# ecmwf-ifs/ecwam

Measured on AMD Instinct MI355X. Metric: grid-point spectral steps/sec (whole node) at O320, 36dir x 36freq, higher is better.
Workload: dtype f32; 1 GPU; O320 all-ocean octahedral grid, 421080 sea points, 36 dir x 36 freq (NFRE_RED=36), full WAMINTGR step = PROPAGS2 advection + NEWWIND + IMPLSCH as one kernel (PROPAGS2 inside IMPLSCH's tile load), IDELT=IDELPRO=450 s, flag set A (IPHYS=1, ISNONLIN=0, LLGCBZ0=F, LLNORMAGAM=F); points_per_gpu=421080, halo_points=0, parallelism=sea-point block x1, ranks=1

## Files before the change

__graft_entry__.py:

```python
from __future__ import annotations

import os
import sys

ROOT = os.path.dirname(os.path.abspath(__file__))
if ROOT not in sys.path:
    sys.path.insert(0, ROOT)


def build() -> None:
    from ecwam_amd import build as b

    lib = b.build()
    assert os.path.exists(lib)
    assert os.path.exists(b.build(variant="ctustrict"))
    assert os.path.exists(b.build(variant="nolead"))
    assert os.path.exists(b.build(variant="notrim"))
    for exe in b.build_fortran():
        assert os.path.exists(exe)
    from oracle import oracle

    oracle.build()
    from oracle import ref_build

    ref_build.build()
    sys.path.insert(0, os.path.join(ROOT, "tests"))
    try:
        import v2lib

        v2lib.build()
    except Exception as e:
        print(f"[build] tests/csrc second implementation not built: {e}", file=sys.stderr)
    import ecwam_amd
    from ecwam_amd import lib as L

    h = L.load()
    for name in L.EXPORTS + L.EXPORTS_START + L.EXPORTS_FORCING + L.EXPORTS_GRIBOUT + L.EXPORTS_GRIBIN:
        getattr(h, name)


def smoke() -> None:
    import numpy as np
    import torch

    sys.path.insert(0, os.path.join(ROOT, "tests"))
    from ecwam_amd import grid as G
    from ecwam_amd.tables import Config
    from ecwam_amd.wamintgr import Wamintgr
    from oracle.oracle import Oracle

    assert torch.cuda.is_available(), "smoke() needs a GPU"
    prec = "sp"
    cfg = Config(nang=36, nfre=36, nfre_red=36, idelt=450, idelpro=450)
    g = G.build_grid(12, mask="continents")
    m = Wamintgr(cfg, g, prec, device=0)
    m.init_synthetic(seed=4)
    assert m.build_weights() == 0 and m.fused_available()
    n = g.nsea
    fl = m.fl1.cpu().numpy().copy()
    wv = m.wvprpt.cpu().numpy()
    ff = m.ff.cpu().numpy()[:, :14].copy()
    env = m.ff.cpu().numpy()[:, 14:16].copy()
    o = Oracle(cfg, prec)
    m.step(fused=True)
    torch.cuda.synchronize()
    f3 = o.propags2(g, fl, o.ctu_weights(g, m.cgroup_ext.cpu().numpy(), float(cfg.idelpro)))
    f3[:, :, cfg.nfre_red:] = fl[:, :, cfg.nfre_red:]
    r = o.implsch(f3[:n], wv[:, 0], wv[:, 1], wv[:, 2], wv[:, 3], wv[:, 4], env, ff, np.zeros((n, 15), np.float32))
    got = m.fl1.cpu().numpy()[:n].astype(np.float64)
    want = r["FL1"].astype(np.float64)
    assert np.isfinite(got).all()
    same = m.mij.cpu().numpy() == r["MIJ"]
    assert same.mean() > 0.99
    peak = np.abs(want).max(axis=(1, 2), keepdims=True)
    err = (np.abs(got - want) / peak)[same].max()
    dfim = np.asarray(m.t.DFIM, dtype=np.float64)
    hs_g, hs_w = (4 * np.sqrt((x.sum(1) * dfim).sum(1)) for x in (got, want))
    e_hs = np.max(np.abs(hs_g - hs_w) / np.maximum(hs_w, 1e-12))
    assert err < 3e-5 and e_hs < 2e-6, (err, e_hs)
    print(f"smoke ok: {n} sea points, one WAMINTGR step as one kernel, max bin error {err:.2e} of the spectral peak, swh {e_hs:.2e}")
    m.ctx.close()


if __name__ == "__main__":
    build()
    if "--smoke" in sys.argv:
        smoke()
```

ecwam_amd/build.py:

```python
from __future__ import annotations

import hashlib
import os
import re
import shutil
import subprocess
import sys

HERE = os.path.dirname(os.path.abspath(__file__))
CSRC = os.path.join(HERE, "csrc")
LIBDIR = os.path.join(HERE, "lib")
LIB = os.path.join(LIBDIR, "libecwam_hip.so")
SOURCES = ["capi.hip", "propag.hip", "implsch4.hip", "implsch4a.hip", "implsch4x.hip", "implsch4r.hip", "implsch4rd.hip", "implsch4w.hip", "outbs.hip", "outbs_sep.hip", "outbs_ext.hip", "outbs_fl2nd.hip", "outbs_2nd.hip", "outbs_int.hip", "outblock.hip", "nest.hip", "start.hip", "forcing.hip", "gribout.hip", "gribin.hip"]
DERIVED = {"implsch4r.hip": ("implsch4r.hip", ["-DV4R_PREC=1"]), "implsch4rd.hip": ("implsch4r.hip", ["-DV4R_PREC=2"])}
HIPCC = shutil.which("hipcc") or "/opt/rocm/bin/hipcc"
FAST_DIV = ["-fno-hip-fp32-correctly-rounded-divide-sqrt"]
FLAGS = ["--offload-arch=gfx950", "-O3", "-fPIC", "-std=c++17", "-Wall", "-Wno-unused-variable", "-Wno-unused-but-set-variable"]
IMPLSCH_SOURCES = ("implsch4.hip", "implsch4a.hip", "implsch4x.hip", "implsch4r.hip", "implsch4rd.hip", "implsch4w.hip")
VARIANTS = {"": FAST_DIV, "exactdiv": ["-DECWAM_HIP_STRICT=0"], "strict1": ["-DECWAM_HIP_STRICT=1"], "strict2": FAST_DIV + ["-DECWAM_HIP_STRICT=2"],
            "site4": ["-DECWAM_HIP_STRICT=4"], "site8": ["-DECWAM_HIP_STRICT=8"], "site32": ["-DECWAM_HIP_STRICT=32"],
            "strict3": ["-DECWAM_HIP_STRICT=3"], "strict7": ["-DECWAM_HIP_STRICT=3", "-ffp-contract=off"],
            "noieee": FAST_DIV + ["-mno-amdgpu-ieee", "-fno-honor-nans"],
            "ctustrict": FAST_DIV,
            "nolead": FAST_DIV + ["-DV4_SINPUT_LEAD=0"],
            "notrim": FAST_DIV + ["-DV4_ONCE_TRIM=0"],
            "advO1": FAST_DIV + ["-O1"]}
VARIANT_ANY = {"ctustrict": ["-DECWAM_HIP_CTU_STRICT=1"]}
VARIANT_SOURCES = {"ctustrict": ("propag.hip", "implsch4a.hip"), "advO1": ("implsch4a.hip",)}

INCLUDE = os.path.join(HERE, "..", "include", "ecwam_hip.h")


def lib_path(variant: str = "") -> str:
    return LIB if not variant else os.path.join(LIBDIR, f"libecwam_hip_{variant}.so")


def _closure(path: str, seen: dict) -> None:
    path = os.path.normpath(path)
    if path in seen or not os.path.exists(path):
        return
    with open(path, "rb") as fh:
        data = fh.read()
    seen[path] = data
    for m in re.finditer(rb'^[ \t]*#[ \t]*include[ \t]*"([^"]+)"', data, re.M):
        _closure(os.path.join(os.path.dirname(path), m.group(1).decode()), seen)


def _stamp(src: str, flags: list) -> str:
    seen: dict = {}
    _closure(os.path.join(CSRC, src), seen)
    h = hashlib.sha256(" ".join([HIPCC, *flags]).encode())
    for k in sorted(seen):
        h.update(os.path.relpath(k, HERE).encode())
        h.update(seen[k])
    return h.hexdigest()


def build(force: bool = False, verbose: bool = False, variant: str = "") -> str:
    if variant not in VARIANTS:
        raise ValueError(f"unknown build variant {variant!r}: {sorted(VARIANTS)}")
    os.makedirs(LIBDIR, exist_ok=True)
    lib = lib_path(variant)
    objs, procs, stamps = [], [], {}
    for src in SOURCES:
        special = bool(variant) and src in VARIANT_SOURCES.get(variant, IMPLSCH_SOURCES)
        obj = os.path.join(LIBDIR, src.replace(".hip", f".{variant}.o" if special else ".o"))
        real_src, extra = DERIVED.get(src, (src, []))
        flags = FLAGS + extra + ((VARIANTS[variant] if special else FAST_DIV) if src in IMPLSCH_SOURCES else []) + (VARIANT_ANY.get(variant, []) if special else [])
        objs.append(obj)
        st = _stamp(real_src, flags)
        old = ""
        if os.path.exists(obj) and os.path.exists(obj + ".stamp"):
            with open(obj + ".stamp") as fh:
                old = fh.read().strip()
        if not force and old == st:
            continue
        stamps[obj] = st
        cmd = [HIPCC, *flags, f"-cuid=ecwam_{os.path.basename(obj).replace('.', '_')}", "-c", os.path.join(CSRC, real_src), "-o", obj]
        if verbose:
            print(" ".join(cmd), flush=True)
        procs.append((src, obj, subprocess.Popen(cmd, stdout=subprocess.PIPE, stderr=subprocess.STDOUT, text=True)))
    for src, obj, p in procs:
        out, _ = p.communicate()
        if p.returncode != 0:
            raise RuntimeError(f"hipcc failed for {src}:\n{out}")
        with open(obj + ".stamp", "w") as fh:
            fh.write(stamps[obj])
        if verbose and out.strip():
            print(out)
    link_stamp = hashlib.sha256("".join(open(o + ".stamp").read() for o in objs).encode()).hexdigest()
    if not procs and os.path.exists(lib) and os.path.exists(lib + ".stamp") and open(lib + ".stamp").read().strip() == link_stamp:
        return lib
    cmd = [HIPCC, "--offload-arch=gfx950", "-shared", "-fPIC", "-Wl,--no-undefined", "-o", lib, *objs]
    r = subprocess.run(cmd, stdout=subprocess.PIPE, stderr=subprocess.STDOUT, text=True)
    if r.returncode != 0:
        raise RuntimeError(f"link failed:\n{r.stdout}")
    with open(lib + ".stamp", "w") as fh:
        fh.write(link_stamp)
    return lib


FLANG = shutil.which("amdflang") or "/opt/rocm/lib/llvm/bin/flang"
FSRC = os.path.join(HERE, "fortran")
FFILES = ["ecwam_hip_capi.F90", "yowdrvtype_hip.F90", "ecwam_hip_mod.F90", "ecwam_hip_restart.F90", "wamintgr_hip.F90", "harness_case.F90"]
FPROGS = {"smoke_wamintgr_hip": "smoke_wamintgr_hip.F90", "seam_sequence": "seam_sequence.F90"}


def fortran_exe(prec: str, prog: str = "smoke_wamintgr_hip") -> str:
    return os.path.join(LIBDIR, f"{prog}_{prec}")


def build_fortran(force: bool = False) -> list:
    build(force=False)
    out = []
    for prec in ("sp", "dp"):
        exes = [fortran_exe(prec, p) for p in FPROGS]
        out += exes
        srcs = [os.path.join(FSRC, f) for f in FFILES + list(FPROGS.values())]
        if not force and all(os.path.exists(e) and all(os.path.getmtime(s) < os.path.getmtime(e) for s in srcs + [LIB]) for e in exes):
            continue
        moddir = os.path.join(LIBDIR, f"fmod_{prec}")
        os.makedirs(moddir, exist_ok=True)
        defs = ["-DECWAM_HIP_SINGLE"] if prec == "sp" else []

        def compile_(s):
            o = os.path.join(moddir, os.path.basename(s).replace(".F90", ".o"))
            r = subprocess.run([FLANG, "-cpp", "-O2", "-fPIC", *defs, "-module-dir", moddir, "-I", moddir, "-c", s, "-o", o],
                               stdout=subprocess.PIPE, stderr=subprocess.STDOUT, text=True)
            if r.returncode != 0:
                raise RuntimeError(f"flang failed for {s}:\n{r.stdout}")
            return o

        objs = [compile_(os.path.join(FSRC, f)) for f in FFILES]
        for prog, f in FPROGS.items():
            po = compile_(os.path.join(FSRC, f))
            r = subprocess.run([FLANG, "-o", fortran_exe(prec, prog), po, *objs, "-L", LIBDIR, "-lecwam_hip", f"-Wl,-rpath,{LIBDIR}", "-Wl,-rpath,$ORIGIN"],
                               stdout=subprocess.PIPE, stderr=subprocess.STDOUT, text=True)
            if r.returncode != 0:
                raise RuntimeError(f"fortran link failed ({prog}):\n{r.stdout}")
    return out


if __name__ == "__main__":
    vs = [a.split("=", 1)[1] for a in sys.argv[1:] if a.startswith("--variant=")]
    for v in vs or [""]:
        print(build(force="--force" in sys.argv, verbose=True, variant=v))
    if not vs:
        print(build_fortran(force="--force" in sys.argv))
```

ecwam_amd/csrc/implsch_v4.h:

```cpp
#pragma once
#include "ctu.h"

#define V4_NFRE 36
#ifdef ECWAM_HIP_DIAGNOSTICS
#define V4_PHASE_EXIT(k) do { if (tb.DBG_SKIP == (k)) return; } while (0)
#else
#define V4_PHASE_EXIT(k) do { } while (0)
#endif
#if defined(V4_CHECK) && V4_CHECK
#include <cassert>
#define V4_CHK(c) assert(c)
#else
#define V4_CHK(c) do { } while (0)
#endif
#ifndef V4_SINPUT_LEAD
#define V4_SINPUT_LEAD 1
#endif
#ifndef V4_ONCE_TRIM
#define V4_ONCE_TRIM 1
#endif
#define V4_NSTG 4
#define V4_NS(nang) ((V4_NFRE + (nang) / 2 - 1) / ((nang) / 2))
#define V4_PLN(pp, nang) ((pp) * ((nang) > V4_NFRE ? (nang) : V4_NFRE))
#define V4_NFAC 6

#define V4SYNC() WSYNC()
#define V4_WPE_MIN(T) (sizeof(T) == 4 ? 2 : 1)

template <typename T>
using V2 = T __attribute__((ext_vector_type(2)));

enum { FIN_AIRD = 0, FIN_UFRIC, FIN_Z0M, FIN_MIJ, FIN_XS, FIN_YS, FIN_F1DCOS3, FIN_F1DCOS2, FIN_F1DSIN2, FIN_F1D, FIN_RNFAC, FIN_PHIWA,
       FIN_SINWD, FIN_COSWD, FIN_WSWAVE, FIN_CICOVER, FIN_PHILF, FIN_XSTRESS, FIN_YSTRESS, FIN_Z0B, FIN_CHRNCK, FIN_COSDIFF, FIN_EMEAN, FIN_F1MEAN,
       FIN_TAUICX, FIN_TAUICY, FIN_STRNMS,
       FIN_W3RT,
       FIN_FMEAN, FIN_FMEANWS, FIN_AKMEAN, FIN_XKMEAN, FIN_SDS, FIN_SC, V4_NFIN = 36 };

__device__ __forceinline__ float v4_bp(int addr, float v) { return __int_as_float(__builtin_amdgcn_ds_bpermute(addr, __float_as_int(v))); }
__device__ __forceinline__ double v4_bp(int addr, double v) {
  const int lo = __builtin_amdgcn_ds_bpermute(addr, __double2loint(v));
  const int hi = __builtin_amdgcn_ds_bpermute(addr, __double2hiint(v));
  return __hiloint2double(hi, lo);
}
template <typename T>
__device__ __forceinline__ V2<T> v4_same(V2<T> v, int addr) {
  V2<T> r;
  r.x = v4_bp(addr, v.x);
  r.y = v4_bp(addr, v.y);
  return r;
}
template <typename T>
struct V4Rot { int a0, a1, a2, a3, a4; T fold; };
template <int CTRL>
__device__ __forceinline__ float v4_dpp(float v) {
  return __int_as_float(__builtin_amdgcn_update_dpp(0, __float_as_int(v), CTRL, 0xf, 0xf, true));
}
template <int CTRL>
__device__ __forceinline__ double v4_dpp(double v) {
  const int lo = __builtin_amdgcn_update_dpp(0, __double2loint(v), CTRL, 0xf, 0xf, true);
  const int hi = __builtin_amdgcn_update_dpp(0, __double2hiint(v), CTRL, 0xf, 0xf, true);
  return __hiloint2double(hi, lo);
}
#define V4_ROW_ROR(n) (0x120 + (n))
template <typename T>
__device__ __forceinline__ V2<T> v4_rowsum(V2<T> v) {
  T x = v.x, y = v.y;
  x += v4_dpp<V4_ROW_ROR(8)>(x); y += v4_dpp<V4_ROW_ROR(8)>(y);
  x += v4_dpp<V4_ROW_ROR(4)>(x); y += v4_dpp<V4_ROW_ROR(4)>(y);
  x += v4_dpp<V4_ROW_ROR(2)>(x); y += v4_dpp<V4_ROW_ROR(2)>(y);
  x += v4_dpp<V4_ROW_ROR(1)>(x); y += v4_dpp<V4_ROW_ROR(1)>(y);
  return V2<T>{x, y};
}
template <typename T>
__device__ __forceinline__ T v4_rowmax(T v) {
  v = m_max(v, v4_dpp<V4_ROW_ROR(8)>(v));
  v = m_max(v, v4_dpp<V4_ROW_ROR(4)>(v));
  v = m_max(v, v4_dpp<V4_ROW_ROR(2)>(v));
  v = m_max(v, v4_dpp<V4_ROW_ROR(1)>(v));
  return v;
}
template <>
__device__ __forceinline__ float v4_rowmax<float>(float v) {
  asm volatile("s_nop 1\n\tv_max_f32_dpp %0, %0, %0 row_ror:8 row_mask:0xf bank_mask:0xf bound_ctrl:1\n\t"
               "s_nop 1\n\tv_max_f32_dpp %0, %0, %0 row_ror:4 row_mask:0xf bank_mask:0xf bound_ctrl:1\n\t"
               "s_nop 1\n\tv_max_f32_dpp %0, %0, %0 row_ror:2 row_mask:0xf bank_mask:0xf bound_ctrl:1\n\t"
               "s_nop 1\n\tv_max_f32_dpp %0, %0, %0 row_ror:1 row_mask:0xf bank_mask:0xf bound_ctrl:1"
               : "+v"(v));
  return v;
}
template <int G, typename T>
__device__ __forceinline__ V2<T> v4_allsum(V2<T> v, const V4Rot<T>& r) {
  if constexpr (G == 18) {
    v = v + r.fold * v4_same<T>(v, r.a0);
    v = v4_rowsum<T>(v);
    return v4_same<T>(v, r.a1);
  } else {
    v = v + v4_same<T>(v, r.a0);
    if (G >= 12) v = v + v4_same<T>(v, r.a1);
    if (G == 24) v = v + v4_same<T>(v, r.a2);
    v = v + (v4_same<T>(v, r.a3) + v4_same<T>(v, r.a4));
    return v;
  }
}
template <int G, typename T>
__device__ __forceinline__ T v4_allsum1(T v, const V4Rot<T>& r) {
  if constexpr (G == 18) {
    v = v + r.fold * v4_bp(r.a0, v);
    v = v + v4_dpp<V4_ROW_ROR(8)>(v);
    v = v + v4_dpp<V4_ROW_ROR(4)>(v);
    v = v + v4_dpp<V4_ROW_ROR(2)>(v);
    v = v + v4_dpp<V4_ROW_ROR(1)>(v);
    return v4_bp(r.a1, v);
  } else {
    v = v + v4_bp(r.a0, v);
    if (G >= 12) v = v + v4_bp(r.a1, v);
    if (G == 24) v = v + v4_bp(r.a2, v);
    v = v + (v4_bp(r.a3, v) + v4_bp(r.a4, v));
    return v;
  }
}

template <int G, int N, int NB, typename T>
__device__ __forceinline__ void v4_allsum_n(T (&v)[N], const V4Rot<T>& r) {
  T e[N];
  if constexpr (G == 18) {
#pragma unroll
    for (int i = 0; i < N; i++) e[i] = v4_bp(r.a0, v[i]);
#pragma unroll
    for (int i = 0; i < N; i++) v[i] = v[i] + r.fold * e[i];
#pragma unroll
    for (int i = 0; i < N; i++) v[i] = v[i] + v4_dpp<V4_ROW_ROR(8)>(v[i]);
#pragma unroll
    for (int i = 0; i < N; i++) v[i] = v[i] + v4_dpp<V4_ROW_ROR(4)>(v[i]);
#pragma unroll
    for (int i = 0; i < N; i++) v[i] = v[i] + v4_dpp<V4_ROW_ROR(2)>(v[i]);
#pragma unroll
    for (int i = 0; i < N; i++) v[i] = v[i] + v4_dpp<V4_ROW_ROR(1)>(v[i]);
#pragma unroll
    for (int i = 0; i < NB; i++) e[i] = v4_bp(r.a1, v[i]);
#pragma unroll
    for (int i = 0; i < NB; i++) v[i] = e[i];
  } else {
#pragma unroll
    for (int i = 0; i < N; i++) e[i] = v4_bp(r.a0, v[i]);
#pragma unroll
    for (int i = 0; i < N; i++) v[i] = v[i] + e[i];
    if constexpr (G >= 12) {
#pragma unroll
      for (int i = 0; i < N; i++) e[i] = v4_bp(r.a1, v[i]);
#pragma unroll
      for (int i = 0; i < N; i++) v[i] = v[i] + e[i];
    }
    if constexpr (G == 24) {
#pragma unroll
      for (int i = 0; i < N; i++) e[i] = v4_bp(r.a2, v[i]);
#pragma unroll
      for (int i = 0; i < N; i++) v[i] = v[i] + e[i];
    }
    T f[N];
#pragma unroll
    for (int i = 0; i < N; i++) { e[i] = v4_bp(r.a3, v[i]); f[i] = v4_bp(r.a4, v[i]); }
#pragma unroll
    for (int i = 0; i < N; i++) v[i] = v[i] + (e[i] + f[i]);
  }
}

template <int G, typename T>
__device__ __forceinline__ T v4_allmax1(T v, const V4Rot<T>& r) {
  if constexpr (G == 18) {
    v = m_max(v, v4_bp(r.a0, v));
    v = v4_rowmax<T>(v);
    return v4_bp(r.a1, v);
  } else {
    v = m_max(v, v4_bp(r.a0, v));
    if (G >= 12) v = m_max(v, v4_bp(r.a1, v));
    if (G == 24) v = m_max(v, v4_bp(r.a2, v));
    return m_max(v, m_max(v4_bp(r.a3, v), v4_bp(r.a4, v)));
  }
}

template <int G, bool UNI, typename T>
__device__ __forceinline__ T v4_uni(T v, int p) {
  if constexpr (UNI && G != 18) return v4_bp(4 * (p * G), v);
  else return v;
}

template <int G, typename T, bool UNI = false>
__device__ __forceinline__ void v4_row_total_to_lds(T v, const V4Rot<T>& r, T* spw, int m, int p = 0) {
  if constexpr (G == 18) {
    v = v + r.fold * v4_bp(r.a0, v);
    v = v + v4_dpp<V4_ROW_ROR(8)>(v);
    v = v + v4_dpp<V4_ROW_ROR(4)>(v);
    v = v + v4_dpp<V4_ROW_ROR(2)>(v);
    v = v + v4_dpp<V4_ROW_ROR(1)>(v);
  } else {
    v = v4_allsum1<G, T>(v, r);
  }
  spw[m] = v4_uni<G, UNI>(v, p);
}

template <typename T, int NSH, int r>
__device__ __forceinline__ V2<T> v4_at(const T* row, const int (&sh)[2 * NSH + 1]) {
  if constexpr ((r & 1) == 0) {
    return *reinterpret_cast<const V2<T>*>(row + sh[r / 2 + NSH]);
  } else {
    return V2<T>{row[sh[(r - 1) / 2 + NSH] + 1], row[sh[(r + 1) / 2 + NSH]]};
  }
}

template <bool ON, typename T>
__device__ __forceinline__ T v4_vreg(T x) {
  if constexpr (ON && sizeof(T) == 4) {
    T r;
    asm("v_mov_b32 %0, %1" : "=v"(r) : "s"(x));
    return r;
  } else return x;
}
template <typename T>
__device__ __forceinline__ void v4_pin6(const T (&r)[6]) { asm volatile("" :: "s"(r[0]), "s"(r[1]), "s"(r[2]), "s"(r[3]), "s"(r[4]), "s"(r[5])); }
template <typename T>
__device__ __forceinline__ void v4_pin10(T (&r)[20], int o) {
  asm volatile("" :: "s"(r[o]), "s"(r[o + 1]), "s"(r[o + 2]), "s"(r[o + 3]), "s"(r[o + 4]), "s"(r[o + 5]), "s"(r[o + 6]), "s"(r[o + 7]), "s"(r[o + 8]), "s"(r[o + 9]));
}
template <typename T, int NSH, int ra, int rb>
__device__ __forceinline__ V2<T> v4_win(const T* row, const int (&sh)[2 * NSH + 1], V2<T> own, T ca, T cb) {
  static_assert(ra - rb == 1 || rb - ra == 1, "adjacent rotations");
  constexpr int lo = ra < rb ? ra : rb;
  constexpr int e = (lo >= 0) ? (lo / 2) * 2 : -(((-lo) + 1) / 2) * 2;
  static_assert(e / 2 + NSH >= 0 && e / 2 + 1 + NSH <= 2 * NSH, "shift table");
  const V2<T> a = (e == 0) ? own : *reinterpret_cast<const V2<T>*>(row + sh[e / 2 + NSH]);
  const V2<T> b = (e + 2 == 0) ? own : *reinterpret_cast<const V2<T>*>(row + sh[e / 2 + 1 + NSH]);
  const T el[4] = {a.x, a.y, b.x, b.y};
  return V2<T>{ca * el[ra - e] + cb * el[rb - e], ca * el[ra - e + 1] + cb * el[rb - e + 1]};
}

template <typename T, int NSH, int r>
__device__ __forceinline__ V2<T> v4_pair(const V2<T> (&A)[2 * NSH + 1]) {
  static_assert(r >= -2 * NSH && r <= 2 * NSH, "window");
  if constexpr ((r & 1) == 0) return A[NSH + r / 2];
  else return __builtin_shufflevector(A[NSH + (r - 1) / 2], A[NSH + (r + 1) / 2], 1, 2);
}
template <typename T, int NSH, int NH, int d>
__device__ __forceinline__ void v4_sat_taps(const V2<T> (&A)[2 * NSH + 1], const T (&wt)[NH + 1], V2<T>& acc) {
  if constexpr (d <= NH) {
    acc += wt[NH - d] * (v4_pair<T, NSH, -d>(A) + v4_pair<T, NSH, d>(A));
    v4_sat_taps<T, NSH, NH, d + 1>(A, wt, acc);
  }
}

template <typename T, int PP, bool RARE>
__device__ __forceinline__ void v4_stresso(const DevTab<T>& tb, T* sSC, int lane, bool LLPHIWA) {
  if constexpr (PP <= 3) {
    stresso_stage<T, PP, RARE>(tb, sSC, lane, LLPHIWA);
  } else {
    stresso_stage<T, 3, RARE>(tb, sSC, lane, LLPHIWA);
    WSYNC();
    v4_stresso<T, PP - 3, RARE>(tb, sSC + 3 * NSC, lane, LLPHIWA);
  }
}

template <typename T, int NANG_, int PP_>
struct V4Ctx {
  int lane, p, j;
  T* tile;
  int own;
  T* fac4;
  T* sq;
  T* zcn;
  T* c;
  V4Rot<T> rot;
  V2<T> sinth, costh;
  T rDFIM, rDFIMOFR, rDFIMFR, rZPIFR, rRHOWG, rCOFRM4, rFLMAX;
};
enum { Q4_BSC = 0, Q4_SBO, Q4_CINV, Q4_WAVNUM };

template <typename T>
struct V4Adv {
  const T* f_in;
  const int* klon;
  const int* klat;
  const int* kcor;
  const T* cg;
  const T* pt;
  const T* dirT;
  const int* dirI;
  T xdella, delpro;
  const T* gin;
  T delpro_lf;
  int gin_k, mlf;
  const T* obs;
  int m0, m1;
};
template <typename T, int NANG, int PP, int MODE, int NSCR>
__device__ __forceinline__ void v4_advect_tile(const V4Adv<T>& A, int ij0, int n, int lane, T* __restrict__ sT, T* __restrict__ sScr) {
  constexpr int NFRE = V4_NFRE, N = NANG * NFRE, RS = PP * NANG, VEC = 16 / (int)sizeof(T), NC = NFRE / VEC, NVL = N / VEC;
  constexpr int NFULL = NVL / 64, NREM = NVL - 64 * NFULL, NTS = (PP * NREM + 63) / 64, NCH = NFULL * PP + NTS, NRND = NFULL + NTS, D = 3;
  constexpr int PTW = 20;
  typedef T VT __attribute__((ext_vector_type(VEC)));
  typedef int I4 __attribute__((ext_vector_type(4)));
  T* sB = sScr;
  T* sPt = sB + PP * 5 * NFRE;
  T* sK = sPt + PP * PTW;
  constexpr bool LF = (MODE & 3) == 3;
  constexpr bool OBS = (MODE & 4) != 0;
  constexpr int NB = OBS ? 11 : 8;
  static_assert(MODE & 1, "modes: 1 plain, 3 fast waves, + 4 obstructions");
  constexpr int NKW = NANG * 4 + 4 + (LF ? NANG * 2 : 0);
  int* sI = reinterpret_cast<int*>(sK + NKW);
  int* sD = sI + PP * 16;
  static_assert((PP * 5 * NFRE + PP * PTW + NKW) * sizeof(T) + (PP * 16 + NANG * 4) * sizeof(int) <= NSCR * sizeof(T), "LDS scratch of the advecting load");
  for (int i = lane; i < PP * PTW; i += 64) {
    const int q = i / PTW, e = i - q * PTW;
    const T* g = A.pt + (size_t)(ij0 + (q < n ? q : n - 1)) * 12;
    T v = T(0);
    if (e < 12) v = g[e];
    else if (e < 18) v = T(1) - g[e - 6];
    else if (e == 18) v = g[0] * g[2];
    else v = A.xdella * g[2];
    if (e == 1) v = m_abs(v);
    sPt[i] = v;
  }
  for (int i = lane; i < PP * 16; i += 64) {
    const int q = i >> 4, e = i & 15;
    const int ijq = ij0 + (q < n ? q : n - 1);
    int v = ijq;
    if (e >= 1 && e <= 2) v = A.klon[(size_t)ijq * 2 + (e - 1)];
    if (e >= 3 && e <= 6) v = A.klat[(size_t)ijq * 4 + (e - 3)];
    if (e >= 7 && e <= 14) v = A.kcor[(size_t)ijq * 8 + (e - 7)];
    sI[i] = v;
  }
  for (int i = lane; i < NKW; i += 64) {
// ... 187 lines not shown
      const T ZLOG2X = ZLOG * ZLOG * X;
      const T GAM_W = ZLOG2X * ZLOG2X * m_exp(XLOG) * tb.OM3GMKM_GC[I];
      const T ZN = CONST * tb.XKMSQRTVGOC2_GC[I] * GAM_W;
      const T GAMNORMA = (T(1) + tb.RN1_RN * ZN) / (T(1) + ZN);
      const T wt = (I == NS) ? tb.DELKCC_GC_NS[NS] * tb.OMXKM3_GC[NS] : tb.DELKCC_OMXKM3_GC[I];
      acc = acc + (GAM_W * wt) * GAMNORMA;
    }
  }
  const T TAUWCG = v4_rowsum<T>(V2<T>{acc, T(0)}).x;
  return m_max(ZABHRC * TAUWCG, TAUWCG_MIN);
}
template <typename T>
__device__ void taut_z0_b_rows(const DevTab<T>& tb, int l16, int IUSFG, T HALP, T UTOP, T COSDIFF, T TAUW, T RNFAC, T& USTAR, T& Z0, T& Z0B,
                               T& CHRNCK) {
  const int NITER = 18;
  const T PMAX = T(0.99), Z0MIN = T(0.000001);
  const T US2TOTAUW = T(1) + tb.EPS1;
  const T RNUKAPPAM1 = (T(0.04) * tb.RNU) / tb.XKAPPA;
  const T PCE_GC = T(0.001) * IUSFG + (1 - IUSFG) * T(0.005);
  const T TAUWACT = m_max(TAUW * COSDIFF, tb.EPSMIN);
  const bool LLCOSDIFF = (COSDIFF > T(0.9));
  T ALPHAOG = T(0);
  if (tb.LLCAPCHNK) ALPHAOG = chnkmin(tb, UTOP) * tb.GM1;
  const T USMAX = m_max(-T(0.21339) + T(0.093698) * UTOP - T(0.0020944) * UTOP * UTOP + T(5.5091E-5) * UTOP * UTOP * UTOP, T(0.03));
  const T TAUWEFF = m_min(TAUWACT * US2TOTAUW, USMAX * USMAX);
  T X, CDFG;
  if (IUSFG == 0) {
    const T ALPHAGM1 = tb.ALPHA * tb.GM1;
    if (UTOP < T(1)) CDFG = T(0.002);
    else if (LLCOSDIFF) {
      const T um = m_max(USTAR, tb.EPSUS);
      X = m_min(TAUWACT / (um * um), PMAX);
      T ZCHAR = m_min(ALPHAGM1 * USTAR * USTAR / m_sqrt(T(1) - X), T(0.05) * m_exp(-T(0.05) * (UTOP - T(35.))));
      ZCHAR = m_min(ZCHAR, tb.ALPHAMAX);
      CDFG = tb.ACDLIN + tb.BCDLIN * m_sqrt(ZCHAR) * UTOP;
    } else CDFG = cdm_d(UTOP);
    USTAR = UTOP * m_sqrt(CDFG);
  }
  const T W1 = T(0.85) - T(0.05) * (m_tanh(T(10) * (UTOP - T(5))) + T(1));
  const T XKUTOP = tb.XKAPPA * UTOP;
  T USTOLD = USTAR;
  T TAUOLD = USTOLD * USTOLD;
  T TAUUNR = T(0);
  bool run = true;
  for (int ITER = 1; ITER <= NITER; ITER++) {
    if (__builtin_amdgcn_ballot_w64(run) == 0ull) break;
    const T Z0n = m_max(tb.XNLEV / (m_exp(m_min(XKUTOP / USTOLD, T(50))) - T(1)), Z0MIN);
    const T TAUV = RNUKAPPAM1 * USTOLD / Z0n;
    const T ANG_GC = tb.ANG_GC_A + tb.ANG_GC_B * m_tanh(tb.ANG_GC_C * TAUOLD);
    const T TAUUNRn = stress_gc_row(tb, l16, run, ANG_GC, USTAR, Z0n, Z0MIN, HALP, RNFAC);
    const T TAUNEW = TAUWEFF + TAUV + TAUUNRn;
    const T USTNEW = m_sqrt(TAUNEW);
    const T USTARn = W1 * USTOLD + (T(1) - W1) * USTNEW;
    if (run) {
      Z0 = Z0n; TAUUNR = TAUUNRn; USTAR = USTARn;
      if (m_abs(USTAR - USTOLD) < PCE_GC * USTAR) run = false;
      else { TAUOLD = USTAR * USTAR; USTOLD = USTAR; }
    }
  }
  X = TAUWEFF / TAUOLD;
  if (run && X >= PMAX) {
    CDFG = cdm_d(UTOP);
    USTAR = UTOP * m_sqrt(CDFG);
    const T Z0MINRST = USTAR * USTAR * tb.ALPHA * tb.GM1;
    Z0 = m_max(tb.XNLEV / (m_exp(XKUTOP / USTAR) - T(1)), Z0MINRST);
    Z0B = Z0MINRST;
  } else {
    Z0 = m_max(tb.XNLEV / (m_exp(XKUTOP / USTAR) - T(1)), Z0MIN);
    Z0B = Z0 * m_sqrt(TAUUNR / TAUOLD);
  }
  if (X < PMAX) {
    const T USNRF = USTAR, Z0NRF = Z0, Z0BNRF = Z0B;
    USTOLD = USTAR;
    TAUOLD = m_max(USTOLD * USTOLD, TAUWEFF);
    const T ALPOG = m_max(m_min(Z0B / TAUOLD, tb.ALPHAMAX), ALPHAOG);
    int ITER;
    for (ITER = 1; ITER <= NITER; ITER++) {
      X = m_min(TAUWEFF / TAUOLD, PMAX);
      const T USTM1 = T(1) / m_max(USTOLD, tb.EPSUS);
      const T Z0VIS = tb.RNUM * USTM1;
      const T HZ0VISO1MX = T(0.5) * Z0VIS / (T(1) - X);
      Z0B = ALPOG * TAUOLD;
      Z0 = HZ0VISO1MX + m_sqrt(HZ0VISO1MX * HZ0VISO1MX + Z0B * Z0B / (T(1) - X));
      const T XOLOGZ0 = T(1) / m_log(tb.XNLEV / Z0 + T(1));
      const T Fv = USTOLD - XKUTOP * XOLOGZ0;
      const T ZZ = T(2) * USTM1 * (T(3) * Z0B * Z0B + T(0.5) * Z0VIS * Z0 - Z0 * Z0) / (T(2) * Z0 * Z0 * (T(1) - X) - Z0VIS * Z0);
      const T DELF = T(1) - XKUTOP * XOLOGZ0 * XOLOGZ0 * ZZ;
      if (DELF != T(0)) USTAR = USTOLD - Fv / DELF;
      const T TAUNEW = m_max(USTAR * USTAR, TAUWEFF);
      USTAR = m_sqrt(TAUNEW);
      const T DEL = TAUNEW - TAUOLD;
      if (m_abs(DEL) < PCE_GC * TAUOLD) break;
      TAUOLD = TAUNEW;
      USTOLD = USTAR;
    }
    if (ITER > NITER) {
      USTAR = USNRF; Z0 = Z0NRF; Z0B = Z0BNRF;
      const T USTM1 = T(1) / m_max(USTAR, tb.EPSUS);
      const T Z0VIS = tb.RNUM * USTM1;
      CHRNCK = m_max(tb.G * (Z0 - Z0VIS) * USTM1 * USTM1, tb.ALPHAMIN);
    } else {
      const T um = m_max(USTAR, tb.EPSUS);
      CHRNCK = m_max(tb.G * (Z0B / m_sqrt(T(1) - X)) / (um * um), tb.ALPHAMIN);
    }
  } else {
    const T USTM1 = T(1) / m_max(USTAR, tb.EPSUS);
    const T Z0VIS = tb.RNUM * USTM1;
    CHRNCK = m_max(tb.G * (Z0 - Z0VIS) * USTM1 * USTM1, tb.ALPHAMIN);
  }
}

template <typename T, int NANG, int PP, int NGST, bool LLSNEG, bool UNI = false>
__device__ void v4_sinput(const DevTab<T>& tb, const V4Ctx<T, NANG, PP>& L, T UFRIC, T Z0M, T RAORW, T SIG_N, T TEMP2, T PTURB, T AIRD_PVISC,
                          T sinwd, T coswd, T* __restrict__ gfl, T* __restrict__ gsp, unsigned long long& xm0, unsigned long long& xm1, V2<T>& wse,
                          V2<T>& wslast, V2<T>& apl, T (&rX)[V4_NS(NANG)], T (&rY)[V4_NS(NANG)], T* __restrict__ sXY) {
  constexpr int G = NANG / 2, NFRE = V4_NFRE, RS = PP * NANG, NS = V4_NS(NANG);
  const T CONST1 = tb.BETAMAXOXKAPPA2, ABS_TAUWSHELTER = m_abs(tb.TAUWSHELTER);
  const T FU = m_abs(tb.SWELLF3), FUD = tb.SWELLF2, ROGOROAIR = tb.G / RAORW;
  const T AVG = T(1) / T(NGST);
  for (int m = L.j; m < NFRE; m += G) L.zcn[m] = m_log(L.fac4[m * 4 + Q4_WAVNUM] * Z0M);
  WSYNC();
  const T XKAPPA = tb.XKAPPA, ZALP = tb.ZALP;
  V2<T> vUSTP = (NGST == 1) ? V2<T>{UFRIC, UFRIC} : V2<T>{UFRIC * (T(1) + SIG_N), UFRIC * (T(1) - SIG_N)};
  V2<T> vXS = {T(0), T(0)}, vYS = {T(0), T(0)};
  const V2<T> vTAUX = (vUSTP * vUSTP) * sinwd, vTAUY = (vUSTP * vUSTP) * coswd;
  xm0 = 0ull; xm1 = 0ull;
  const V2<T> z2 = {T(0), T(0)};
  wse = z2; wslast = z2; apl = z2;
#pragma unroll
  for (int s = 0; s < NS; s++) { rX[s] = T(0); rY[s] = T(0); }
  const T* tF = L.tile + L.own;
  constexpr bool LEAD = (V4_SINPUT_LEAD != 0) && sizeof(T) == 4;
  int m0 = 0;
  if constexpr (LEAD) {
    const V2<T> vTPX = vTAUX - ABS_TAUWSHELTER * vXS, vTPY = vTAUY - ABS_TAUWSHELTER * vYS;
    const V2<T> vh2 = vTPX * vTPX + vTPY * vTPY;
    const T TINY = sizeof(T) == 4 ? T(1e-36) : T(1e-300);
    V2<T> vrh = {fs_rsq<8>(m_max(vh2.x, TINY)), (NGST == 2) ? fs_rsq<8>(m_max(vh2.y, TINY)) : T(0)};
    if (NGST == 1) vrh.y = vrh.x;
    const V2<T> vh = vh2 * vrh, vCOSU = vTPY * vrh, vSINU = vTPX * vrh;
    V2<T> vUSTP0 = V2<T>{fs_sqrt<8>(vh.x), (NGST == 2) ? fs_sqrt<8>(vh.y) : T(0)};
    if (NGST == 1) vUSTP0.y = vUSTP0.x;
    V2<T> rcl[NGST], ds2[NGST];
    bool c0[NGST], c1[NGST];
#pragma unroll
    for (int ig = 0; ig < NGST; ig++) {
      const T COSU = ig ? vCOSU.y : vCOSU.x, SINU = ig ? vSINU.y : vSINU.x;
      const T USTPg = ig ? vUSTP0.y : vUSTP0.x;
      const V2<T> coslp = L.costh * COSU + L.sinth * SINU;
      c0[ig] = coslp.x > T(0.01); c1[ig] = coslp.y > T(0.01);
      rcl[ig] = V2<T>{fs_rcp<4>(coslp.x), fs_rcp<4>(coslp.y)};
      ds2[ig] = LLSNEG ? TEMP2 + (FU + FUD * coslp) * USTPg : z2;
    }
    {
      T ci_n = L.fac4[Q4_CINV], zcn_l = L.zcn[0];
#pragma unroll 1
      for (; m0 < NFRE; m0++) {
        const T cinv_m = ci_n, ZCN = zcn_l;
        const int mn = m0 + 1 < NFRE ? m0 + 1 : m0;
        ci_n = L.fac4[mn * 4 + Q4_CINV];
        zcn_l = L.zcn[mn];
        const V2<T> vUCN = vUSTP0 * cinv_m;
        const V2<T> vden = vUCN + ZALP;
        const V2<T> vUZ = XKAPPA * V2<T>{fs_rcp<8>(vden.x), (NGST == 2) ? fs_rcp<8>(vden.y) : T(0)};
        bool grows = false;
#pragma unroll
        for (int ig = 0; ig < NGST; ig++) {
          const T UCNZALPD = ig ? vUZ.y : vUZ.x;
          const T Z0 = ZCN + UCNZALPD * rcl[ig].x, Z1 = ZCN + UCNZALPD * rcl[ig].y;
          const bool n0 = c0[ig] && (Z0 < T(0)), n1 = c1[ig] && (Z1 < T(0));
          grows = grows || n0 || n1;
        }
        if (__builtin_amdgcn_ballot_w64(grows) != 0ull) break;
      }
    }
    static_assert(NFRE % 2 == 0, "the row loop takes its rows in pairs");
    m0 = m0 < NFRE ? (m0 & ~1) : NFRE - 2;
    if constexpr (G == 18) {
      for (int m = 0; m < m0; m++) *reinterpret_cast<V2<T>*>(sXY + 2 * m) = z2;
    }
    if constexpr (LLSNEG) {
      if (m0 > 0) {
        const int lr = L.lane < NFRE ? L.lane : NFRE - 1;
        const T k2 = tb.SINROW[lr][2], k3 = tb.SINROW[lr][3], k4 = tb.SINROW[lr][4];
        V2<T> f_l = *reinterpret_cast<const V2<T>*>(tF);
        T wn_l = L.fac4[Q4_CINV + 1];
#pragma unroll 1
        for (int m = 0; m < m0; m++) {
          const V2<T> f = f_l;
          const T wavnum_m = wn_l;
          const int mn = m + 1 < NFRE ? m + 1 : m;
          f_l = *reinterpret_cast<const V2<T>*>(tF + mn * RS);
          wn_l = L.fac4[mn * 4 + Q4_CINV + 1];
          const T row2 = __int_as_float(__builtin_amdgcn_readlane(__float_as_int(k2), m));
          const T row3 = __int_as_float(__builtin_amdgcn_readlane(__float_as_int(k3), m));
          const T row4 = __int_as_float(__builtin_amdgcn_readlane(__float_as_int(k4), m));
          const T DSTAB1 = (row2 * AIRD_PVISC) * wavnum_m;
          const T TEMP1 = row3 * RAORW;
          V2<T> FLP[NGST];
#pragma unroll
          for (int ig = 0; ig < NGST; ig++) {
            const V2<T> DSTAB2 = TEMP1 * ds2[ig];
            const V2<T> dstab = DSTAB1 + PTURB * DSTAB2;
            FLP[ig] = z2 + dstab;
          }
          V2<T> fl = FLP[0];
          if (NGST == 2) fl = fl + FLP[NGST - 1];
          fl = AVG * fl;
          apl = apl + (fl * f - z2) * row4;
          *reinterpret_cast<V2<T>*>(gfl + (size_t)m * NANG) = fl;
          gsp[m] = T(0);
        }
      }
    }
  }
  const int mp = LEAD ? 2 * (int)((unsigned)m0 >> 1) : 0;
  V2<T> f_n = *reinterpret_cast<const V2<T>*>(tF + mp * RS);
  V2<T> cw_n = *reinterpret_cast<const V2<T>*>(L.fac4 + mp * 4 + Q4_CINV);
  T zcn_n = L.zcn[mp];
  constexpr bool RPF = sizeof(T) == 4;
  T rw_n[6];
  if constexpr (RPF) {
#pragma unroll
    for (int i = 0; i < 6; i++) rw_n[i] = tb.SINROW[mp][i];
  }
#pragma unroll 2
  for (int m = mp; m < NFRE; m++) {
    const V2<T> f = f_n, cw = cw_n;
    const T ZCN = zcn_n, cinv_m = cw.x;
    T rw[6];
    if constexpr (RPF) {
#pragma unroll
      for (int i = 0; i < 6; i++) rw[i] = rw_n[i];
    }
    {
      const int mn = m + 1 < NFRE ? m + 1 : m;
      f_n = *reinterpret_cast<const V2<T>*>(tF + mn * RS);
      cw_n = *reinterpret_cast<const V2<T>*>(L.fac4 + mn * 4 + Q4_CINV);
      zcn_n = L.zcn[mn];
      if constexpr (RPF) {
#pragma unroll
        for (int i = 0; i < 6; i++) rw_n[i] = tb.SINROW[mn][i];
      }
    }
    if constexpr (RPF) __builtin_amdgcn_sched_barrier(0);
    V4_CHK(m >= 0 && m < NFRE);
    const T* row = RPF ? rw : tb.SINROW[m];
    const T SIGm = row[0], DFIMm = row[1];
    const T CONSTF = ROGOROAIR * cinv_m * DFIMm;
    const T DSTAB1 = LLSNEG ? (row[2] * AIRD_PVISC) * cw.y : T(0);
    const T CNSN = (SIGm * CONST1) * RAORW;
    const T TEMP1 = LLSNEG ? row[3] * RAORW : T(0);
    V2<T> SLP[2], FLP[2];
    bool xl0 = false, xl1 = false;
    const V2<T> vTPX = vTAUX - ABS_TAUWSHELTER * vXS, vTPY = vTAUY - ABS_TAUWSHELTER * vYS;
    const V2<T> vh2 = vTPX * vTPX + vTPY * vTPY;
    const T TINY = sizeof(T) == 4 ? T(1e-36) : T(1e-300);
    V2<T> vrh = {fs_rsq<8>(m_max(vh2.x, TINY)), (NGST == 2) ? fs_rsq<8>(m_max(vh2.y, TINY)) : T(0)};
    if (NGST == 1) vrh.y = vrh.x;
    const V2<T> vh = vh2 * vrh, vCOSU = vTPY * vrh, vSINU = vTPX * vrh;
    vUSTP = V2<T>{fs_sqrt<8>(vh.x), (NGST == 2) ? fs_sqrt<8>(vh.y) : T(0)};
    if (NGST == 1) vUSTP.y = vUSTP.x;
    const V2<T> vUCN = vUSTP * cinv_m;
    const V2<T> vden = vUCN + ZALP;
    const V2<T> vUZ = XKAPPA * V2<T>{fs_rcp<8>(vden.x), (NGST == 2) ? fs_rcp<8>(vden.y) : T(0)};
#pragma unroll
    for (int ig = 0; ig < NGST; ig++) {
      const T COSU = ig ? vCOSU.y : vCOSU.x, SINU = ig ? vSINU.y : vSINU.x;
      const T UCN = ig ? vUCN.y : vUCN.x, UCNZALPD = ig ? vUZ.y : vUZ.x;
      const T USTPg = ig ? vUSTP.y : vUSTP.x;
      const V2<T> coslp = L.costh * COSU + L.sinth * SINU;
      V2<T> gam0 = z2;
      {
        const bool c0 = coslp.x > T(0.01), c1 = coslp.y > T(0.01);
        const T Z0 = ZCN + UCNZALPD * fs_rcp<4>(coslp.x), Z1 = ZCN + UCNZALPD * fs_rcp<4>(coslp.y);
        const bool n0 = c0 && (Z0 < T(0)), n1 = c1 && (Z1 < T(0));
        if (sizeof(T) == 4 || __builtin_amdgcn_ballot_w64(n0 || n1) != 0ull) {
          const V2<T> ZL = {Z0, Z1};
          const V2<T> Z2X = ZL * ZL * (coslp * UCN);
          const V2<T> ex = {f_exp(Z0), f_exp(Z1)};
          const V2<T> g = ex * Z2X * Z2X * CNSN;
          gam0.x = n0 ? g.x : T(0);
          gam0.y = n1 ? g.y : T(0);
          xl0 = xl0 || n0;
          xl1 = xl1 || n1;
        }
      }
      V2<T> dstab = z2;
      if (LLSNEG) {
        const V2<T> DSTAB2 = TEMP1 * (TEMP2 + (FU + FUD * coslp) * USTPg);
        dstab = DSTAB1 + PTURB * DSTAB2;
      }
      FLP[ig] = gam0 + dstab;
      SLP[ig] = gam0 * f;
    }
    V2<T> sp = SLP[0], fl = FLP[0];
    if (NGST == 2) { sp = sp + SLP[1]; fl = fl + FLP[1]; }
    sp = AVG * sp;
    fl = AVG * fl;
    T xrow = T(0), yrow = T(0);
    constexpr bool REDN = sizeof(T) == 4;
    if constexpr (REDN) {
      constexpr int NR = 2 * NGST + (LLSNEG ? 1 : 0);
      T red[NR];
#pragma unroll
      for (int ig = 0; ig < NGST; ig++) {
        const V2<T> sx = SLP[ig] * L.sinth, sy = SLP[ig] * L.costh;
// ... 1593 lines not shown
```

Before: 63.45 million grid-point spectral steps/s.

## Parallelize SINPUT growth-threshold frequency search across lanes with ballot

Replaces the serial per-frequency loop that finds the first growing frequency in the wind input with a lane-parallel search. Each lane takes one frequency per stage, the minimum reciprocal cosine is reduced across directions with DPP min, and a wave ballot plus count-trailing-zeros picks the first frequency. This removes a sequential dependent loop of reciprocals in favour of a few stages of wide work. It adds inline DPP assembly and cross-lane reductions, and it relies on the min-rcl reformulation giving the same threshold. A nopar build variant is added for comparison.

```diff
diff --git a/__graft_entry__.py b/__graft_entry__.py
--- a/__graft_entry__.py
+++ b/__graft_entry__.py
@@ -15,6 +15,7 @@
     assert os.path.exists(lib)
     assert os.path.exists(b.build(variant="ctustrict"))
     assert os.path.exists(b.build(variant="nolead"))
+    assert os.path.exists(b.build(variant="nopar"))
     assert os.path.exists(b.build(variant="notrim"))
     for exe in b.build_fortran():
         assert os.path.exists(exe)
diff --git a/ecwam_amd/build.py b/ecwam_amd/build.py
--- a/ecwam_amd/build.py
+++ b/ecwam_amd/build.py
@@ -23,6 +23,7 @@
             "noieee": FAST_DIV + ["-mno-amdgpu-ieee", "-fno-honor-nans"],
             "ctustrict": FAST_DIV,
             "nolead": FAST_DIV + ["-DV4_SINPUT_LEAD=0"],
+            "nopar": FAST_DIV + ["-DV4_SINPUT_PAR=0"],
             "notrim": FAST_DIV + ["-DV4_ONCE_TRIM=0"],
             "advO1": FAST_DIV + ["-O1"]}
 VARIANT_ANY = {"ctustrict": ["-DECWAM_HIP_CTU_STRICT=1"]}
diff --git a/ecwam_amd/csrc/implsch_v4.h b/ecwam_amd/csrc/implsch_v4.h
--- a/ecwam_amd/csrc/implsch_v4.h
+++ b/ecwam_amd/csrc/implsch_v4.h
@@ -16,6 +16,9 @@
 #ifndef V4_SINPUT_LEAD
 #define V4_SINPUT_LEAD 1
 #endif
+#ifndef V4_SINPUT_PAR
+#define V4_SINPUT_PAR 1
+#endif
 #ifndef V4_ONCE_TRIM
 #define V4_ONCE_TRIM 1
 #endif
@@ -177,6 +180,37 @@
     if (G == 24) v = m_max(v, v4_bp(r.a2, v));
     return m_max(v, m_max(v4_bp(r.a3, v), v4_bp(r.a4, v)));
   }
+}
+
+template <int G>
+__device__ __forceinline__ float v4_allmin1(float v, const V4Rot<float>& r) {
+  if constexpr (G == 18) {
+    v = m_min(v, v4_bp(r.a0, v));
+    asm volatile("s_nop 1\n\tv_min_f32_dpp %0, %0, %0 row_ror:8 row_mask:0xf bank_mask:0xf bound_ctrl:1\n\t"
+                 "s_nop 1\n\tv_min_f32_dpp %0, %0, %0 row_ror:4 row_mask:0xf bank_mask:0xf bound_ctrl:1\n\t"
+                 "s_nop 1\n\tv_min_f32_dpp %0, %0, %0 row_ror:2 row_mask:0xf bank_mask:0xf bound_ctrl:1\n\t"
+                 "s_nop 1\n\tv_min_f32_dpp %0, %0, %0 row_ror:1 row_mask:0xf bank_mask:0xf bound_ctrl:1"
+                 : "+v"(v));
+    return v4_bp(r.a1, v);
+  } else {
+    v = m_min(v, v4_bp(r.a0, v));
+    if (G >= 12) v = m_min(v, v4_bp(r.a1, v));
+    if (G == 24) v = m_min(v, v4_bp(r.a2, v));
+    return m_min(v, m_min(v4_bp(r.a3, v), v4_bp(r.a4, v)));
+  }
+}
+template <int G, int PP>
+__device__ __forceinline__ int v4_first_j(unsigned long long mask) {
+  unsigned f = 0u;
+  if constexpr (G == 18) {
+    const unsigned e = (unsigned)(mask >> 48) & 0x3fu;
+    f = (((unsigned)mask | (unsigned)(mask >> 16) | (unsigned)(mask >> 32)) & 0xffffu) | (((e | (e >> 2) | (e >> 4)) & 3u) << 16);
+  } else {
+    static_assert(PP * G <= 64, "one wave");
+#pragma unroll
+    for (int q = 0; q < PP; q++) f |= (unsigned)(mask >> (q * G)) & ((1u << G) - 1u);
+  }
+  return f ? __builtin_ctz(f) : -1;
 }
 
 template <int G, bool UNI, typename T>
@@ -670,7 +704,32 @@
       rcl[ig] = V2<T>{fs_rcp<4>(coslp.x), fs_rcp<4>(coslp.y)};
       ds2[ig] = LLSNEG ? TEMP2 + (FU + FUD * coslp) * USTPg : z2;
     }
-    {
+    if constexpr ((V4_SINPUT_PAR != 0) && sizeof(T) == 4 && ECWAM_HIP_STRICT == 0) {
+      T rmin[NGST];
+#pragma unroll
+      for (int ig = 0; ig < NGST; ig++) {
+        const T PINF = __builtin_huge_valf();
+        rmin[ig] = v4_allmin1<G>(m_min(c0[ig] ? rcl[ig].x : PINF, c1[ig] ? rcl[ig].y : PINF), L.rot);
+      }
+      m0 = NFRE;
+#pragma unroll
+      for (int s = NS - 1; s >= 0; s--) {
+        const int mr = s * G + L.j;
+        const bool in = (NS * G == NFRE) || mr < NFRE;
+        const int mi = in ? mr : NFRE - 1;
+        const T cinv_m = L.fac4[mi * 4 + Q4_CINV], ZCN = L.zcn[mi];
+        bool grows = false;
+#pragma unroll
+        for (int ig = 0; ig < NGST; ig++) {
+          const T den = __builtin_fmaf(ig ? vUSTP0.y : vUSTP0.x, cinv_m, ZALP);
+          const T UCNZALPD = XKAPPA * fs_rcp<8>(den);
+          const T Z = __builtin_fmaf(UCNZALPD, rmin[ig], ZCN);
+          grows = grows || (Z < T(0));
+        }
+        const int jf = v4_first_j<G, PP>(__builtin_amdgcn_ballot_w64(grows && in));
+        m0 = jf >= 0 ? s * G + jf : m0;
+      }
+    } else {
       T ci_n = L.fac4[Q4_CINV], zcn_l = L.zcn[0];
 #pragma unroll 1
       for (; m0 < NFRE; m0++) {
```

New measurement: 64.78 million grid-point spectral steps/s, median of 6. 2.1% higher.
